# VladimirP1/rs-sync

Hardware: NVIDIA B200
Metric: presync_loss_evals_per_s (higher is better)
Workload: dtype f64

## Files before the change

rs-sync_b200/csrc/capi.cpp:

```cpp
#include "rssync_b200.h"

#include <algorithm>
#include <atomic>
#include <chrono>
#include <cmath>
#include <condition_variable>
#include <cstdio>
#include <cstdlib>
#include <cstring>
#include <functional>
#include <map>
#include <mutex>
#include <string>
#include <thread>
#include <unordered_set>
#include <utility>
#include <vector>
#if defined(__x86_64__)
#include <immintrin.h>
#endif
#if defined(__linux__)
#include <pthread.h>
#include <sched.h>
#endif
// ... 206 lines not shown
    DevBuf<unsigned> d_var_flags;
    size_t elim_n = 0;

    std::vector<rssync_problem*> replicas;
    std::vector<void*> comms;
    bool is_replica = false, owns_stream = false;
    bool force_single = false;
    uint64_t version = 0, synced_version = 0;
    DevBuf<unsigned char> d_gather;
    PinBuf<unsigned char> h_gather;
    uint64_t nccl_calls = 0, broadcast_bytes = 0;

    DevBuf<FrameDesc> d_frames;
    DevBuf<double> d_delays, d_framecost, d_costs;
    DevBuf<unsigned> d_flags;
    DevBuf<rs::PixelFrame> d_pixframes;
    DevBuf<uint64_t> d_frame_call;
    DevBuf<int> d_win_begin;
    PinBuf<double> h_pix;
    DevBuf<double> d_pix, d_stage;
    PinBuf<double> h_stage;
    std::vector<SyncLane> lanes;
    cudaEvent_t ev_sync_ready = nullptr;
    DevBuf<double> d_probe;

    std::unordered_map<int64_t, std::pair<double, double>> retime;
    DevBuf<double> d_rowq;
    DevBuf<double> d_rt_rays, d_rt_ext;
    DevBuf<int32_t> d_rt_orig, d_rt_pos;

// ... 145 lines not shown
    return RSSYNC_OK;
}

int check_grid_size(rssync_problem* p, long long F, long long D) {
    if (F * D > (1LL << 34)) { p->err = "pre-sync: grid too large"; return RSSYNC_E_INVALID; }
    return RSSYNC_OK;
}

int stage_grid(rssync_problem* p, const FrameDesc* frames, size_t n_frames, int F, const double* delays, int D,
               int curves) {
    CUDA_TRY(p, p->d_frames.reserve(std::max<size_t>(n_frames, 1)));
    CUDA_TRY(p, p->d_delays.reserve((size_t)D));
    CUDA_TRY(p, p->d_framecost.reserve((size_t)std::max(F, 1) * D));
    CUDA_TRY(p, p->d_costs.reserve((size_t)curves * D));
    CUDA_TRY(p, p->d_flags.reserve((size_t)curves * 2));
    CUDA_TRY(p, cudaMemsetAsync(p->d_flags.ptr, 0, (size_t)curves * 2 * sizeof(unsigned), p->stream));
    if (F == 0) return RSSYNC_OK;
    if (int rc = h2d(p, p->d_frames.ptr, frames, sizeof(FrameDesc) * n_frames)) return rc;
    return h2d(p, p->d_delays.ptr, delays, sizeof(double) * D);
}

int grid_max_chunk(const FrameDesc* frames, int F, const double* delays, int D, double sr, int max_n) {
    double span = 0.0;
    for (int f = 0; f < F; ++f) span = std::max(span, frames[f].ts_hi - frames[f].ts_lo);
    return rs::presync_max_chunk(delays, D, span, sr, max_n);
}

std::vector<uint64_t> call_numbers(const rssync_problem* p, const uint64_t* call_nos, int n) {
    std::vector<uint64_t> calls((size_t)n);
    for (int i = 0; i < n; ++i) calls[(size_t)i] = call_nos ? call_nos[i] : p->call_no + (uint64_t)i;
// ... 110 lines not shown
        run_end.push_back(F);
        if (run_end.size() > 16) { run_end.assign(1, F); run_dep.assign(1, (int)p->in_flight.size()); }
    } else {
        run_end.assign(1, F);
        run_dep.assign(1, 0);
    }
    const rs::DeviceData dd = p->device_data();
    if (timed) CUDA_TRY(p, cudaEventRecord(p->ev0, p->stream));
    int f0 = 0, waited = 0;
    if (run_end.size() == 1) {
        if (run_dep[0] > 0) {
            CUDA_TRY(p, cudaStreamWaitEvent(p->stream, p->in_flight[(size_t)run_dep[0] - 1].ev, 0));
            waited = run_dep[0];
        }
        rs::launch_presync_tasks(dd, p->d_frames.ptr, F, max_n, p->d_delays.ptr, n, p->seed, stream_id, call_no,
                                 idx_base, p->d_framecost.ptr, F, d_flags, p->stream, nullptr, max_chunk, p->simplified);
    } else {
        for (int k = 0; k < rssync_problem::kGridStreams; ++k) {
            if (!p->grid_stream[k]) CUDA_TRY(p, cudaStreamCreateWithFlags(&p->grid_stream[k], cudaStreamNonBlocking));
            if (!p->ev_grid[k]) CUDA_TRY(p, cudaEventCreateWithFlags(&p->ev_grid[k], cudaEventDisableTiming));
        }
        if (!p->ev_order) CUDA_TRY(p, cudaEventCreateWithFlags(&p->ev_order, cudaEventDisableTiming));
        CUDA_TRY(p, cudaEventRecord(p->ev_order, p->stream));
        for (size_t r = 0; r < run_end.size(); ++r) {
            cudaStream_t gs = p->grid_stream[r % rssync_problem::kGridStreams];
            if (r < (size_t)rssync_problem::kGridStreams) CUDA_TRY(p, cudaStreamWaitEvent(gs, p->ev_order, 0));
            if (run_dep[r] > 0) {
                CUDA_TRY(p, cudaStreamWaitEvent(gs, p->in_flight[(size_t)run_dep[r] - 1].ev, 0));
                waited = std::max(waited, run_dep[r]);
            }
            int spare = 0;
            for (size_t k = (size_t)run_dep[r]; k < p->in_flight.size(); ++k)
                if (p->in_flight[k].foreign) spare = spare_sms_for_collectives();
            rs::launch_presync_tasks(dd, p->d_frames.ptr + f0, run_end[r] - f0, max_n, p->d_delays.ptr, n, p->seed,
                                     stream_id, call_no, idx_base, p->d_framecost.ptr + f0, F, d_flags, gs,
                                     nullptr, max_chunk, p->simplified, spare);
            f0 = run_end[r];
        }
        for (int k = 0; k < rssync_problem::kGridStreams; ++k) {
            CUDA_TRY(p, cudaEventRecord(p->ev_grid[k], p->grid_stream[k]));
            CUDA_TRY(p, cudaStreamWaitEvent(p->stream, p->ev_grid[k], 0));
        }
    }
    if (timed) CUDA_TRY(p, cudaEventRecord(p->ev1, p->stream));
    if (n_launches) *n_launches = run_end.size();
    if (n_waited) *n_waited = waited;
    for (int k = 0; k < waited; ++k) p->ev_pool.push_back(p->in_flight[(size_t)k].ev);
    p->in_flight.erase(p->in_flight.begin(), p->in_flight.begin() + waited);
    return RSSYNC_OK;
}

// ... 508 lines not shown
    for (rssync_problem* r : p->replicas) r->synced_version = p->version;
    p->broadcast_bytes += p->nq * 16 * sizeof(double);
    for (const Piece& pc : pieces) p->broadcast_bytes += (pc.hi - pc.lo) * (8 * sizeof(double) + 2 * sizeof(int32_t));
    return RSSYNC_OK;
}

int grid_enqueue_rank(rssync_problem* q, const std::vector<FrameDesc>& sel, int max_n, const double* delays,
                      int cnt, uint64_t stream_id, uint64_t call_no, uint64_t idx_base, int max_chunk,
                      double* d_costs_dst, unsigned* d_flags_dst, bool timed) {
    const int F = (int)sel.size();
    CUDA_TRY(q, cudaMemsetAsync(d_flags_dst, 0, 2 * sizeof(unsigned), q->stream));
    if (cnt <= 0) return RSSYNC_OK;
    CUDA_TRY(q, q->d_frames.reserve(F));
    CUDA_TRY(q, q->d_delays.reserve(cnt));
    CUDA_TRY(q, q->d_framecost.reserve((size_t)F * cnt));
    if (int rc = h2d(q, q->d_frames.ptr, sel.data(), sizeof(FrameDesc) * F)) return rc;
    if (int rc = h2d(q, q->d_delays.ptr, delays, sizeof(double) * cnt)) return rc;
    if (int rc = enqueue_grid_kernels(q, sel, max_n, cnt, stream_id, call_no, idx_base, d_flags_dst, max_chunk, timed,
                                      nullptr, nullptr))
        return rc;
    rs::launch_presync_reduce(q->d_framecost.ptr, F, cnt, d_costs_dst, q->stream);
    CUDA_TRY(q, cudaGetLastError());
    return RSSYNC_OK;
}

int multi_presync_grid(rssync_problem* p, int64_t fb, int64_t fe, const double* delays, int n,
                       uint64_t stream_id, uint64_t call_no, uint64_t idx_base, double* costs,
                       unsigned* flags_out) {
    std::vector<FrameDesc> sel;
    int max_n = 0;
// ... 229 lines not shown
    for (int k = 0; k < rssync_problem::kGridStreams; ++k) {
        if (p->grid_stream[k]) cudaStreamDestroy(p->grid_stream[k]);
        if (p->ev_grid[k]) cudaEventDestroy(p->ev_grid[k]);
    }
    if (p->gyro_stream) { cudaStreamSynchronize(p->gyro_stream); cudaStreamDestroy(p->gyro_stream); }
    if (p->ev_gyro) cudaEventDestroy(p->ev_gyro);
    p->d_rec.release();
    p->h_gyro.release();
    p->d_gyro.release();
    p->h_rays.release(); p->d_rays.release();
    p->h_orig.release(); p->d_orig.release();
    p->h_pos.release(); p->d_pos.release();
    p->d_frames.release(); p->d_delays.release(); p->d_framecost.release(); p->d_costs.release();
    p->d_frame_call.release(); p->d_win_begin.release();
    p->h_pix.release(); p->d_pix.release(); p->d_pixframes.release(); p->d_stage.release();
    p->d_flags.release(); p->h_stage.release(); p->d_probe.release();
    p->d_gather.release(); p->h_gather.release();
    p->d_var_ts.release(); p->d_var_in.release(); p->d_var_q.release(); p->d_var_y.release(); p->d_var_rhs.release();
    p->d_var_rec.release(); p->d_var_prefix.release(); p->d_elim.release();
    p->d_var_orients.release(); p->d_var_flags.release();
    p->d_rowq.release(); p->d_rt_rays.release(); p->d_rt_ext.release(); p->d_rt_orig.release(); p->d_rt_pos.release();
    if (p->owns_stream && p->stream) { cudaStreamSynchronize(p->stream); cudaStreamDestroy(p->stream); }
    for (SyncLane& L : p->lanes) L.release();
    if (p->ev_sync_ready) cudaEventDestroy(p->ev_sync_ready);
    if (p->ev0) cudaEventDestroy(p->ev0);
    if (p->ev1) cudaEventDestroy(p->ev1);
    delete p;
}

const char* rssync_last_error(const rssync_problem* p) { return p ? p->err.c_str() : "null problem"; }

// ... 914 lines not shown
    if (!call_nos) p->call_no += (uint64_t)n;
    if (int rc = flush(p)) return rc;
    const int F = (int)all.size();
    std::vector<double> costs((size_t)n * D, 0.0);
    unsigned flags[2] = {0, 0};
    if (F > 0) {
        if (int rc = check_grid_size(p, F, D)) return rc;
        const int max_chunk = grid_max_chunk(all.data(), F, delays.data(), D, p->sr, max_n);
        if (int rc = stage_grid(p, all.data(), all.size(), F, delays.data(), D, n)) return rc;
        CUDA_TRY(p, p->d_frame_call.reserve(F));
        CUDA_TRY(p, p->d_win_begin.reserve(n + 1));
        if (int rc = h2d(p, p->d_frame_call.ptr, fcall.data(), sizeof(uint64_t) * F)) return rc;
        if (int rc = h2d(p, p->d_win_begin.ptr, wbeg.data(), sizeof(int) * (n + 1))) return rc;
        rs::launch_presync_grid(p->device_data(), p->d_frames.ptr, F, max_n, p->d_delays.ptr, D, p->seed,
                                rs::kStreamPreSync, 0, 0, p->d_framecost.ptr, p->d_costs.ptr, p->d_flags.ptr,
                                p->stream, max_chunk, p->simplified, p->d_frame_call.ptr, p->d_win_begin.ptr, n);
        if (int rc = d2h(p, costs.data(), p->d_costs.ptr, sizeof(double) * n * D)) return rc;
        if (int rc = d2h(p, flags, p->d_flags.ptr, 2 * sizeof(unsigned))) return rc;
        if (int rc = finish_stream(p, p->stream)) return rc;
        p->grid_tasks = (uint64_t)F * (uint64_t)D;
        p->grid_exact_tasks = flags[1];
    }
    if (flags[0]) { p->err = presync_panic_text(flags[0]); return RSSYNC_E_NONFINITE; }
    for (int i = 0; i < n; ++i) curve_argmin(&costs[(size_t)i * D], delays.data(), D, &out_cost[i], &out_delay[i]);
    return RSSYNC_OK;
}

int rssync_debug_presync(rssync_problem* p, double initial, int64_t fb, int64_t fe, double radius,
                         double* delays, double* costs, int point_count) {
    RS_NVTX_RANGE();
    if (!p || (point_count > 0 && (!delays || !costs))) return RSSYNC_E_INVALID;
// ... 135 lines not shown
    for (int k0 = 0; k0 < n_orient; k0 += G) {
        const int g = std::min(G, n_orient - k0);
        rs::launch_gyro_integrate(p->d_var_in.ptr, p->d_var_in.ptr + n, (int)n, &mats[(size_t)k0 * 9], g, p->d_var_orients.ptr,
                                  p->d_var_q.ptr, p->d_var_prefix.ptr, st);
        rs::launch_gyro_resample(p->d_var_ts.ptr, (int)n, p->d_var_q.ptr, g, plan.tick0, plan.rate_hz, (int)nq,
                                 p->d_var_y.ptr, p->d_var_flags.ptr + k0, st);
        rs::launch_spline_chains(p->d_var_y.ptr, p->d_elim.ptr, p->d_elim.ptr + nq, (int)nq, g, p->d_var_rhs.ptr, st);
        for (int v = 0; v < g; ++v) {
            double* rec = p->d_var_rec.ptr + (size_t)v * nq * 16;
            rs::launch_spline_finish(p->d_var_y.ptr + (size_t)v * nq * 4, p->d_var_rhs.ptr + (size_t)v * nq * 4,
                                     p->d_elim.ptr + 2 * nq, (int)nq, rec, st);
            if (F > 0) {
                dd.rec = rec;
                rs::launch_presync_grid(dd, p->d_frames.ptr, F, max_n, p->d_delays.ptr, D, p->seed, rs::kStreamPreSync,
                                        calls[(size_t)(k0 + v)], 0, p->d_framecost.ptr,
                                        p->d_costs.ptr + (size_t)(k0 + v) * D, p->d_flags.ptr + 2 * (size_t)(k0 + v), st,
                                        max_chunk, p->simplified);
            }
        }
        CUDA_TRY(p, cudaGetLastError());
        if (k0 + g >= n_orient) {
            CUDA_TRY(p, p->d_rec.reserve(nq * 16));
            CUDA_TRY(p, cudaMemcpyAsync(p->d_rec.ptr, p->d_var_rec.ptr + (size_t)(g - 1) * nq * 16, nq * 16 * sizeof(double),
                                        cudaMemcpyDeviceToDevice, st));
        }
    }
    std::vector<double> costs((size_t)n_orient * D, 0.0);
    std::vector<unsigned> resampled((size_t)n_orient, 0u), flags((size_t)n_orient * 2, 0u);
    if (F > 0)
        if (int rc = d2h(p, costs.data(), p->d_costs.ptr, costs.size() * sizeof(double))) return rc;
    if (int rc = d2h(p, resampled.data(), p->d_var_flags.ptr, resampled.size() * sizeof(unsigned))) return rc;
    if (int rc = d2h(p, flags.data(), p->d_flags.ptr, flags.size() * sizeof(unsigned))) return rc;
// ... 151 lines not shown
                retimed_bounds(rec[(size_t)f], &ext[(size_t)f * 4], readouts[j], table[f].ts_lo, table[f].ts_hi);
            }
            max_chunk[(size_t)j] = grid_max_chunk(table, F, delays.data(), D, p->sr, max_n);
        }
        if (int rc = stage_grid(p, tables.data(), tables.size(), F, delays.data(), D, n)) return rc;
        rs::DeviceData dd = p->device_data();
        dd.rays = p->d_rt_rays.ptr;
        dd.orig = p->d_rt_orig.ptr;
        dd.pos = p->d_rt_pos.ptr;
        for (int j = 0; j < n; ++j) {
            if (j > 0)
                rs::launch_retime_frames(p->d_pixframes.ptr, F, p->d_rays.ptr, p->d_orig.ptr, p->d_rowq.ptr, readouts[j],
                                         p->d_rt_rays.ptr, p->d_rt_orig.ptr, p->d_rt_pos.ptr, nullptr, st);
            rs::launch_presync_grid(dd, p->d_frames.ptr + (size_t)j * F, F, max_n, p->d_delays.ptr, D, p->seed,
                                    rs::kStreamPreSync, calls[(size_t)j], 0, p->d_framecost.ptr,
                                    p->d_costs.ptr + (size_t)j * D, p->d_flags.ptr + 2 * (size_t)j, st,
                                    max_chunk[(size_t)j], p->simplified);
        }
        if (int rc = d2h(p, costs.data(), p->d_costs.ptr, costs.size() * sizeof(double))) return rc;
        if (int rc = d2h(p, flags.data(), p->d_flags.ptr, flags.size() * sizeof(unsigned))) return rc;
        if (int rc = finish_stream(p, st)) return rc;
        p->grid_tasks = (uint64_t)F * (uint64_t)D;
        p->grid_exact_tasks = flags[(size_t)n * 2 - 1];
    }
    for (int j = 0; j < n; ++j) {
        if (const unsigned fl = flags[2 * (size_t)j]) { p->err = presync_panic_text(fl); return RSSYNC_E_NONFINITE; }
        const double* c = &costs[(size_t)j * D];
        curve_argmin(c, delays.data(), D, &out_cost[j], &out_delay[j]);
        if (out_curves) std::memcpy(out_curves + (size_t)j * D, c, sizeof(double) * D);
    }
    return RSSYNC_OK;
// ... 457 lines not shown
```

rs-sync_b200/csrc/engine.cu:

```cuda
#include "engine.h"

#include <algorithm>
#include <atomic>
#include <cmath>
#include <cstdio>
#include <map>
#include <mutex>
#include <tuple>
#include <utility>
#include <vector>

#include "device_math.cuh"
#include "gyro_scan.h"

namespace rs {

namespace {

constexpr unsigned FULL = 0xffffffffu;

#ifdef RS_CHECKED
__device__ int* g_assert_slot = nullptr;
#define RS_ASSERT(cond)                                                      \
    do {                                                                     \
// ... 860 lines not shown
#ifndef RS_GRID_RECS
#define RS_GRID_RECS 128
#endif
#ifndef RS_LOSS_UNROLL
#define RS_LOSS_UNROLL 4
#endif
#ifndef RS_GRID_GRAB
#define RS_GRID_GRAB 4
#endif
#ifndef RS_GRID_PRIOR
#define RS_GRID_PRIOR 1
#endif
#ifndef RS_PRIOR_BUMP
#define RS_PRIOR_BUMP 0x00800000u
#endif
template <int SLOTS>
struct GridCfg {
    static constexpr int kWarps = RS_GRID_WARPS;
    static constexpr int kMinBlocks = SLOTS <= 8 ? RS_GRID_MINB : 1;
    static constexpr size_t kTileBytes = (size_t)SLOTS * 2048;
    static constexpr long long kRoom = (228 * 1024) / kMinBlocks - 1024 - (long long)kLog1pTableBytes - 256 -
                                       (long long)kWarps * (long long)warp_smem_bytes(SLOTS * 32) - 2 * (long long)kTileBytes;
    static constexpr int kRecsFit = (int)(kRoom / 256 / 8 * 8);
    static constexpr int kRecs = kRecsFit < RS_GRID_RECS ? kRecsFit : RS_GRID_RECS;
    static_assert(kRecs >= 40, "grid kernel: no room for a spline window");
    static constexpr size_t kBufBytes = kTileBytes + (size_t)kRecs * 128;
    static constexpr size_t kCtlOff = kLog1pTableBytes;
    static constexpr size_t kBufOff = kCtlOff + 256;
    static constexpr size_t kWarpOff = kBufOff + 2 * kBufBytes;
    static constexpr size_t kSmem = kWarpOff + (size_t)kWarps * warp_smem_bytes(SLOTS * 32);
    static_assert(kMinBlocks * (kSmem + 1024) <= 228 * 1024, "grid kernel: shared memory over budget");
};
struct GridCtl {
    unsigned long long full[2];
    int done_a[2];
    int next_task;
    int rec_first[2], rec_cnt[2];
    int frame[2], d0[2];
    int unit[2];
    FrameDesc fd[2];
};
static_assert(sizeof(GridCtl) <= 256, "GridCtl must fit its slot");

__device__ __noinline__ void grid_stage_unit(const DeviceData& dd, const FrameDesc* frames,
                                             const double* delays, int D, int chunk, int fi, int ci, int u,
                                             GridCtl* ctl, int b, double* sTiles, double* sRec, int rec_cap) {
    const int d0 = ci * chunk;
    const int d1 = min(D, d0 + chunk);
    const FrameDesc fd = frames[fi];
    double dmin = delays[d0], dmax = dmin;
    for (int d = d0 + 1; d < d1; ++d) {
        dmin = fmin(dmin, delays[d]);
        dmax = fmax(dmax, delays[d]);
    }
    const double x_lo = ((fd.ts_lo - dd.q0) + dmin) * dd.sr, x_hi = ((fd.ts_hi - dd.q0) + dmax) * dd.sr;
    const double r_lo = floor(x_lo) - 1.0, r_hi = floor(x_hi) + 2.0;
    const bool ok = dd.sr > 0.0 && r_lo >= 0.0 && r_hi <= (double)(dd.nq - 1) && (r_hi - r_lo) < (double)rec_cap;
    const int first = ok ? (int)r_lo : 0, cnt = ok ? (int)(r_hi - r_lo) + 1 : 0;
    ctl->rec_first[b] = first;
    ctl->rec_cnt[b] = cnt;
    ctl->frame[b] = fi;
    ctl->d0[b] = d0;
    ctl->fd[b] = fd;
    __threadfence_block();
    *(volatile int*)&ctl->unit[b] = u;
    asm volatile("fence.proxy.async.shared::cta;" ::: "memory");
    const unsigned tile_bytes = (unsigned)((fd.n + 31) >> 5) * 2048u;
    const unsigned bytes = ok ? (unsigned)cnt * 128u + tile_bytes : 0u;
    mbar_arrive_expect_tx(&ctl->full[b], bytes);
    if (ok) {
        tma_load_1d(sRec, dd.rec + (size_t)first * 16, (unsigned)cnt * 128u, &ctl->full[b]);
        tma_load_1d(sTiles, dd.rays + (size_t)fd.off * 8, tile_bytes, &ctl->full[b]);
    }
}

template <int SLOTS, bool SIMPLE>
__global__ void __launch_bounds__(GridCfg<SLOTS>::kWarps * 32, GridCfg<SLOTS>::kMinBlocks)
presync_kernel(DeviceData dd, const FrameDesc* __restrict__ frames, int F,
               const double* __restrict__ delays, int D, int chunk, int cpf, uint64_t seed,
               uint64_t stream, uint64_t call_no, const uint64_t* __restrict__ frame_call_no,
               uint64_t idx_base, double* __restrict__ framecost, int cost_stride,
               unsigned* __restrict__ flags, int staged) {
    using Cfg = GridCfg<SLOTS>;
    constexpr bool simplified = SIMPLE;
    extern __shared__ __align__(128) unsigned char smem_raw[];
    constexpr int NP = SLOTS * 32;
    const int lane = threadIdx.x & 31, warp = threadIdx.x >> 5;
    double* tab = reinterpret_cast<double*>(smem_raw);
    GridCtl* ctl = reinterpret_cast<GridCtl*>(smem_raw + Cfg::kCtlOff);
    unsigned char* bufs = smem_raw + Cfg::kBufOff;
    const WarpSmem w = warp_smem(smem_raw + Cfg::kWarpOff, warp, NP);
    const long long U = (long long)F * cpf;
    const long long u_begin = U * blockIdx.x / gridDim.x;
    const int n_units = (int)(U * (blockIdx.x + 1) / gridDim.x - u_begin);
    const int fi0 = (int)(u_begin / cpf), c0 = (int)(u_begin % cpf);
    auto stage = [&](int u) {
        const int cu = c0 + u, b = u & 1;
        double* sTiles = reinterpret_cast<double*>(bufs + (size_t)b * Cfg::kBufBytes);
        grid_stage_unit(dd, frames, delays, D, chunk, fi0 + cu / cpf, cu % cpf, u, ctl, b, sTiles,
                        sTiles + SLOTS * 256, Cfg::kRecs);
    };
    if (threadIdx.x == 0) {
        mbar_init(&ctl->full[0], 1);
        mbar_init(&ctl->full[1], 1);
        ctl->done_a[0] = ctl->done_a[1] = 0;
        ctl->unit[0] = ctl->unit[1] = -1;
        ctl->next_task = 0;
        asm volatile("fence.mbarrier_init.release.cluster;" ::: "memory");
    }
    load_log1p_table(tab);
    if (threadIdx.x == 0 && staged) {
        if (n_units > 0) stage(0);
        if (n_units > 1) stage(1);
    }
    const int n_tasks = n_units * chunk;
    int cur_u = -1, rec_first = 0, rec_cnt = 0, fi = 0, d0 = 0;
    FrameDesc fd{};
    unsigned prior = 0u;
    int prior_u = -1, prior_dj = -2;
    for (int k_next = 0, k_end = 0;;) {
        if (k_next == k_end) {
            if (lane == 0) k_next = atomicAdd(&ctl->next_task, RS_GRID_GRAB);
            k_next = __shfl_sync(FULL, k_next, 0);
            k_end = min(k_next + RS_GRID_GRAB, n_tasks);
            if (k_next >= n_tasks) break;
        }
        const int k = k_next++;
        const int u = k / chunk, dj = k - u * chunk;
        const int b = u & 1;
        if (u != cur_u && !staged) {
            cur_u = u;
            const int cu = c0 + u;
            fi = fi0 + cu / cpf;
            d0 = (cu % cpf) * chunk;
            fd = frames[fi];
        } else if (u != cur_u) {
            cur_u = u;
#ifdef RS_CHECKED
            unsigned spins = 0;
#endif
            for (int have; (have = *(volatile int*)&ctl->unit[b]) != u;) {
                RS_ASSERT(++spins < (1u << 24) && have < u);
                __nanosleep(RS_POLL_NS);
            }
            const unsigned parity = (unsigned)(u >> 1) & 1u;
            while (!mbar_try_wait(&ctl->full[b], parity)) {
                RS_ASSERT(++spins < (1u << 24));
                __nanosleep(RS_POLL_NS);
            }
            RS_ASSERT(*(volatile int*)&ctl->unit[b] == u);
            rec_first = *(volatile int*)&ctl->rec_first[b];
            rec_cnt = *(volatile int*)&ctl->rec_cnt[b];
            fi = *(volatile int*)&ctl->frame[b];
            d0 = *(volatile int*)&ctl->d0[b];
            const volatile FrameDesc* vf = &ctl->fd[b];
            fd.id = vf->id; fd.off = vf->off; fd.n = vf->n; fd.ts_lo = vf->ts_lo; fd.ts_hi = vf->ts_hi;
        }
        const int di = d0 + dj;
        const bool active = di < D;
        RS_ASSERT(fi >= 0 && fi < F && dj >= 0 && dj < chunk && fd.n >= 2 && fd.n <= NP);
        double delay = 0.0;
        if (active) {
            delay = delays[di];
            const double* sTiles = reinterpret_cast<const double*>(bufs + (size_t)b * Cfg::kBufBytes);
            if (rec_cnt) build_rows_staged(dd, fd, delay, lane, w, NP, sTiles, sTiles + SLOTS * 256, rec_first, rec_cnt);
            else build_rows_global_cold(dd, fd, delay, lane, w, NP);
        }
        __syncwarp();
        if (lane == 0 && staged) {
            __threadfence_block();
            RS_ASSERT(*(volatile int*)&ctl->unit[b] == u);
            const int done = atomicAdd(&ctl->done_a[b], 1);
            RS_ASSERT(done >= 0 && done < chunk);
            if (done == chunk - 1) {
                ctl->done_a[b] = 0;
                if (u + 2 < n_units) stage(u + 2);
            }
        }
        if (!active) continue;
        const uint64_t key =
            rng_task_key(rng_prefix(seed, stream, frame_call_no ? frame_call_no[fi] : call_no,
                                    idx_base + (uint64_t)di),
                         fd.id);
        double M[3] = {0.0, 0.0, 0.0};
        unsigned bad = 0u;
        if (!simplified) {
            const bool neighbour = RS_GRID_PRIOR && prior && prior_u == u && prior_dj + 1 == dj && prior < 0x7e000000u;
            unsigned tau = 0u;
            bad = warp_ransac<SLOTS>(dd, fd, w, 20, key, lane, M, flags + 1, neighbour ? prior + RS_PRIOR_BUMP : 0u,
                                     &tau);
            prior = tau;
            prior_u = u;
            prior_dj = dj;
        }
        __syncwarp();
        constexpr int LU = RS_LOSS_UNROLL < SLOTS ? RS_LOSS_UNROLL : SLOTS;
        double ss = 0.0;
#pragma unroll 1
        for (int s0 = 0; s0 < SLOTS; s0 += LU) {
            double pm[LU];
#pragma unroll
            for (int j = 0; j < LU; ++j) {
                const int i = (s0 + j) * 32 + lane;
                pm[j] = 0.0;
                if (s0 + j < SLOTS) {
                    const double p0 = w.P[i], p1 = w.P[NP + i], p2 = w.P[2 * NP + i];
                    pm[j] = simplified ? sqrt(dot3(p0, p1, p2, p0, p1, p2)) : dot3(p0, p1, p2, M[0], M[1], M[2]);
                    w.P[i] = pm[j];
// ... 13 lines not shown
                const double r = (s0 + j < SLOTS ? w.P[(s0 + j) * 32 + lane] : 0.0) * scale;
                rho[j] = sqrt(log1p_nonneg(r * r, tab));
            }
#pragma unroll
            for (int j = 0; j < LU; ++j) acc = acc + rho[j];
        }
        const double cost = sqrt(warp_sum(acc));
        if (lane == 0) framecost[(size_t)di * cost_stride + fi] = cost;
        if (bad || !is_finite(cost)) {
            if (simplified && !is_finite(ss)) bad |= kFlagP;
            bad |= presync_diagnose(w.P, (fd.n + 31) >> 5, lane, scale, M[0], M[1], M[2], tab);
            bad = __reduce_or_sync(FULL, bad);
            if (bad && lane == 0) atomicOr(flags, bad);
        }
    }
}

__global__ void reduce_rows_kernel(const double* __restrict__ in, int rows, int cols,
                                   double* __restrict__ out) {
    const int lane = threadIdx.x & 31;
    const int row = blockIdx.x * (blockDim.x >> 5) + (threadIdx.x >> 5);
    if (row >= rows) return;
    DD acc = dd_zero();
    for (int c = lane; c < cols; c += 32) dd_add(acc, in[(size_t)row * cols + c]);
    const double v = warp_dd_sum(acc);
    if (lane == 0) out[row] = v;
}

__global__ void reduce_windows_kernel(const double* __restrict__ in, int D, int F,
                                      const int* __restrict__ win_begin, int W,
// ... 721 lines not shown
    int*& h = slots[dev];
    if (!h) {
        cudaHostAlloc((void**)&h, sizeof(int), cudaHostAllocMapped);
        *h = 0;
        int* d = nullptr;
        cudaHostGetDevicePointer((void**)&d, h, 0);
        cudaMemcpyToSymbol(g_assert_slot, &d, sizeof(d));
        return 0;
    }
    return *(volatile int*)h;
#else
    return 0;
#endif
}

uint64_t launch_count() { return g_launches.load(); }
void count_launches(uint64_t n) { g_launches += n; }

int presync_max_chunk(const double* h_delays, int D, double frame_span_s, double sample_rate, int max_n) {
    if (D <= 1) return 1;
    int recs = 0;
    RS_DISPATCH_SLOTS(max_n, { recs = GridCfg<SL>::kRecs; });
    double step = 0.0;
    for (int i = 1; i < D; ++i) step = std::max(step, std::fabs(h_delays[i] - h_delays[i - 1]));
    const double room = ((double)recs - 5.0) / sample_rate - frame_span_s;
    if (!(room > 0.0) || !(step == step)) return 1;
    if (step <= 0.0) return D;
    const double c = std::floor(room / step) + 1.0;
    return (int)std::max(1.0, std::min(c, (double)D));
}

void launch_presync_tasks(const DeviceData& dd, const FrameDesc* d_frames, int F, int max_n,
                          const double* d_delays, int D, uint64_t seed, uint64_t stream, uint64_t call_no,
                          uint64_t idx_base, double* d_framecost, int cost_stride, unsigned* d_flags,
                          cudaStream_t st, const uint64_t* d_frame_call_no, int max_chunk, bool simplified,
                          int spare_sms) {
    if (F <= 0 || D <= 0) return;
    RS_DISPATCH_SLOTS(max_n, {
        using Cfg = GridCfg<SL>;
        auto kern = simplified ? presync_kernel<SL, true> : presync_kernel<SL, false>;
        allow_smem(kern, Cfg::kSmem);
        const int sm_count = sm_count_of(current_device());
        const int per_sm = blocks_per_sm(kern, Cfg::kWarps * 32, Cfg::kSmem);
        const long long blocks_cap = (long long)std::max(1, sm_count - std::max(0, spare_sms)) * per_sm;
        int chunk = std::min(D, max_chunk > 0 ? max_chunk : Cfg::kWarps * 2);
        const long long cpf_par = (blocks_cap * 4 + F - 1) / F;
        const int chunk_par = (int)std::max<long long>(1, (D + cpf_par - 1) / cpf_par);
        chunk = std::min(chunk, std::max(chunk_par, std::min(D, Cfg::kWarps)));
        const int cpf = (D + chunk - 1) / chunk;
        chunk = (D + cpf - 1) / cpf;
        const long long units = (long long)F * cpf;
        const int grid = (int)std::max<long long>(1, std::min<long long>(units, blocks_cap));
        const int staged = chunk >= Cfg::kWarps ? 1 : 0;
        kern<<<grid, Cfg::kWarps * 32, Cfg::kSmem, st>>>(dd, d_frames, F, d_delays, D, chunk, cpf, seed, stream,
                                                         call_no, d_frame_call_no, idx_base, d_framecost,
                                                         cost_stride, d_flags, staged);
    });
    g_launches += 1;
}

void launch_presync_reduce(const double* d_framecost, int F, int D, double* d_costs, cudaStream_t st,
                           const int* d_win_begin, int n_windows) {
    if (D <= 0) return;
    if (F <= 0) {
        cudaMemsetAsync(d_costs, 0, sizeof(double) * D * (d_win_begin ? n_windows : 1), st);
        return;
    }
    if (d_win_begin)
        reduce_windows_kernel<<<(n_windows * D + 3) / 4, 128, 0, st>>>(d_framecost, D, F, d_win_begin,
                                                                      n_windows, d_costs);
    else
        reduce_rows_kernel<<<(D + 3) / 4, 128, 0, st>>>(d_framecost, D, F, d_costs);
    g_launches += 1;
}

void launch_presync_grid(const DeviceData& dd, const FrameDesc* d_frames, int F, int max_n,
                         const double* d_delays, int D, uint64_t seed, uint64_t stream,
                         uint64_t call_no, uint64_t idx_base, double* d_framecost, double* d_costs,
                         unsigned* d_flags, cudaStream_t st, int max_chunk, bool simplified,
                         const uint64_t* d_frame_call_no, const int* d_win_begin, int n_windows) {
    launch_presync_tasks(dd, d_frames, F, max_n, d_delays, D, seed, stream, call_no, idx_base, d_framecost, F,
                         d_flags, st, d_frame_call_no, max_chunk, simplified);
    launch_presync_reduce(d_framecost, F, D, d_costs, st, d_win_begin, n_windows);
}

void launch_sync_init(const DeviceData& dd, const SyncBatchDev& b, const double* d_sp_delay,
                      const uint64_t* d_sp_callno, const unsigned char* d_sp_active, uint64_t seed,
                      cudaStream_t st) {
    if (b.T <= 0) return;
    RS_DISPATCH_SLOTS(b.max_n, {
        auto kern = sync_init_kernel<SL>;
        const size_t smem = (size_t)kWarpsPerBlock * warp_smem_bytes(SL * 32);
        allow_smem(kern, smem);
        const int grid = grid_for(kern, smem, b.T);
        kern<<<grid, kWarpsPerBlock * 32, smem, st>>>(dd, b, d_sp_delay, d_sp_callno, d_sp_active, seed);
    });
    g_launches += 1;
// ... 190 lines not shown
```

rs-sync_b200/csrc/engine.h:

```cpp
#pragma once
#include <cstdint>
#include <cuda_runtime.h>

namespace rs {

constexpr int kMaxRaysPerFrame = 512;
constexpr double kNumericDiffStep = 1e-6;

struct FrameDesc {
    int64_t id;
    int32_t off;
    int32_t n;
    double ts_lo, ts_hi;
};

struct DeviceData {
    const double* rec;
    int nq;
    double q0, sr;
    const double* rays;
    const int32_t* orig;
    const int32_t* pos;
};

enum RngStream : uint64_t { kStreamPreSync = 1, kStreamDebugPreSync = 2, kStreamSyncInit = 3 };

enum : unsigned { kFlagP = 1u, kFlagM = 2u, kFlagR = 4u, kFlagRho = 8u };

void launch_presync_grid(const DeviceData& dd, const FrameDesc* d_frames, int F, int max_n,
                         const double* d_delays, int D, uint64_t seed, uint64_t stream,
                         uint64_t call_no, uint64_t idx_base, double* d_framecost, double* d_costs,
                         unsigned* d_flags, cudaStream_t st, int max_chunk, bool simplified,
                         const uint64_t* d_frame_call_no = nullptr, const int* d_win_begin = nullptr,
                         int n_windows = 0);

int presync_max_chunk(const double* h_delays, int D, double frame_span_s, double sample_rate, int max_n);

void launch_presync_tasks(const DeviceData& dd, const FrameDesc* d_frames, int F, int max_n,
                          const double* d_delays, int D, uint64_t seed, uint64_t stream, uint64_t call_no,
                          uint64_t idx_base, double* d_framecost, int cost_stride, unsigned* d_flags,
                          cudaStream_t st, const uint64_t* d_frame_call_no = nullptr, int max_chunk = 0,
                          bool simplified = false, int spare_sms = 0);
void launch_presync_reduce(const double* d_framecost, int F, int D, double* d_costs, cudaStream_t st,
                           const int* d_win_begin = nullptr, int n_windows = 0);

struct SyncTask {
    FrameDesc fd;
    int32_t sp;
    int32_t pad;
};
struct SyncBatchDev {
    const SyncTask* tasks;
    int T;
    int max_n;
    const int* sp_begin;
    int S;
    double* m;
// ... 83 lines not shown
```

Measured before the change: 33.07 billion.

## Replace static per-block unit split with global atomic work queue for presync grid

The presync kernel no longer gives each block a fixed contiguous range of (frame, chunk) units. Warps now claim units from a device-global atomic counter: whole units first, then a tail split into smaller sub-parts to balance load at the end. Staging also precomputes RNG task keys per unit in shared memory and reduces delay min/max across the warp. The cost is one global atomic per claim, an extra memset per launch, more control shared memory and more complex producer/consumer handshakes.

After: 34.41 billion, median of 6. +4.1%, better.

```diff
diff --git a/rs-sync_b200/csrc/capi.cpp b/rs-sync_b200/csrc/capi.cpp
--- a/rs-sync_b200/csrc/capi.cpp
+++ b/rs-sync_b200/csrc/capi.cpp
@@ -244,6 +244,7 @@
     DevBuf<FrameDesc> d_frames;
     DevBuf<double> d_delays, d_framecost, d_costs;
     DevBuf<unsigned> d_flags;
+    DevBuf<unsigned long long> d_queue;
     DevBuf<rs::PixelFrame> d_pixframes;
     DevBuf<uint64_t> d_frame_call;
     DevBuf<int> d_win_begin;
@@ -419,6 +420,7 @@
     CUDA_TRY(p, p->d_framecost.reserve((size_t)std::max(F, 1) * D));
     CUDA_TRY(p, p->d_costs.reserve((size_t)curves * D));
     CUDA_TRY(p, p->d_flags.reserve((size_t)curves * 2));
+    CUDA_TRY(p, p->d_queue.reserve(1 + rssync_problem::kGridStreams));
     CUDA_TRY(p, cudaMemsetAsync(p->d_flags.ptr, 0, (size_t)curves * 2 * sizeof(unsigned), p->stream));
     if (F == 0) return RSSYNC_OK;
     if (int rc = h2d(p, p->d_frames.ptr, frames, sizeof(FrameDesc) * n_frames)) return rc;
@@ -559,7 +561,8 @@
             waited = run_dep[0];
         }
         rs::launch_presync_tasks(dd, p->d_frames.ptr, F, max_n, p->d_delays.ptr, n, p->seed, stream_id, call_no,
-                                 idx_base, p->d_framecost.ptr, F, d_flags, p->stream, nullptr, max_chunk, p->simplified);
+                                 idx_base, p->d_framecost.ptr, F, d_flags, p->d_queue.ptr, p->stream, nullptr, max_chunk,
+                                 p->simplified);
     } else {
         for (int k = 0; k < rssync_problem::kGridStreams; ++k) {
             if (!p->grid_stream[k]) CUDA_TRY(p, cudaStreamCreateWithFlags(&p->grid_stream[k], cudaStreamNonBlocking));
@@ -568,7 +571,8 @@
         if (!p->ev_order) CUDA_TRY(p, cudaEventCreateWithFlags(&p->ev_order, cudaEventDisableTiming));
         CUDA_TRY(p, cudaEventRecord(p->ev_order, p->stream));
         for (size_t r = 0; r < run_end.size(); ++r) {
-            cudaStream_t gs = p->grid_stream[r % rssync_problem::kGridStreams];
+            const size_t k = r % rssync_problem::kGridStreams;
+            cudaStream_t gs = p->grid_stream[k];
             if (r < (size_t)rssync_problem::kGridStreams) CUDA_TRY(p, cudaStreamWaitEvent(gs, p->ev_order, 0));
             if (run_dep[r] > 0) {
                 CUDA_TRY(p, cudaStreamWaitEvent(gs, p->in_flight[(size_t)run_dep[r] - 1].ev, 0));
@@ -578,8 +582,8 @@
             for (size_t k = (size_t)run_dep[r]; k < p->in_flight.size(); ++k)
                 if (p->in_flight[k].foreign) spare = spare_sms_for_collectives();
             rs::launch_presync_tasks(dd, p->d_frames.ptr + f0, run_end[r] - f0, max_n, p->d_delays.ptr, n, p->seed,
-                                     stream_id, call_no, idx_base, p->d_framecost.ptr + f0, F, d_flags, gs,
-                                     nullptr, max_chunk, p->simplified, spare);
+                                     stream_id, call_no, idx_base, p->d_framecost.ptr + f0, F, d_flags,
+                                     p->d_queue.ptr + 1 + k, gs, nullptr, max_chunk, p->simplified, spare);
             f0 = run_end[r];
         }
         for (int k = 0; k < rssync_problem::kGridStreams; ++k) {
@@ -1118,6 +1122,7 @@
     CUDA_TRY(q, q->d_frames.reserve(F));
     CUDA_TRY(q, q->d_delays.reserve(cnt));
     CUDA_TRY(q, q->d_framecost.reserve((size_t)F * cnt));
+    CUDA_TRY(q, q->d_queue.reserve(1 + rssync_problem::kGridStreams));
     if (int rc = h2d(q, q->d_frames.ptr, sel.data(), sizeof(FrameDesc) * F)) return rc;
     if (int rc = h2d(q, q->d_delays.ptr, delays, sizeof(double) * cnt)) return rc;
     if (int rc = enqueue_grid_kernels(q, sel, max_n, cnt, stream_id, call_no, idx_base, d_flags_dst, max_chunk, timed,
@@ -1377,7 +1382,7 @@
     p->d_frames.release(); p->d_delays.release(); p->d_framecost.release(); p->d_costs.release();
     p->d_frame_call.release(); p->d_win_begin.release();
     p->h_pix.release(); p->d_pix.release(); p->d_pixframes.release(); p->d_stage.release();
-    p->d_flags.release(); p->h_stage.release(); p->d_probe.release();
+    p->d_flags.release(); p->d_queue.release(); p->h_stage.release(); p->d_probe.release();
     p->d_gather.release(); p->h_gather.release();
     p->d_var_ts.release(); p->d_var_in.release(); p->d_var_q.release(); p->d_var_y.release(); p->d_var_rhs.release();
     p->d_var_rec.release(); p->d_var_prefix.release(); p->d_elim.release();
@@ -2322,7 +2327,8 @@
         if (int rc = h2d(p, p->d_win_begin.ptr, wbeg.data(), sizeof(int) * (n + 1))) return rc;
         rs::launch_presync_grid(p->device_data(), p->d_frames.ptr, F, max_n, p->d_delays.ptr, D, p->seed,
                                 rs::kStreamPreSync, 0, 0, p->d_framecost.ptr, p->d_costs.ptr, p->d_flags.ptr,
-                                p->stream, max_chunk, p->simplified, p->d_frame_call.ptr, p->d_win_begin.ptr, n);
+                                p->d_queue.ptr, p->stream, max_chunk, p->simplified, p->d_frame_call.ptr,
+                                p->d_win_begin.ptr, n);
         if (int rc = d2h(p, costs.data(), p->d_costs.ptr, sizeof(double) * n * D)) return rc;
         if (int rc = d2h(p, flags, p->d_flags.ptr, 2 * sizeof(unsigned))) return rc;
         if (int rc = finish_stream(p, p->stream)) return rc;
@@ -2488,8 +2494,8 @@
                 dd.rec = rec;
                 rs::launch_presync_grid(dd, p->d_frames.ptr, F, max_n, p->d_delays.ptr, D, p->seed, rs::kStreamPreSync,
                                         calls[(size_t)(k0 + v)], 0, p->d_framecost.ptr,
-                                        p->d_costs.ptr + (size_t)(k0 + v) * D, p->d_flags.ptr + 2 * (size_t)(k0 + v), st,
-                                        max_chunk, p->simplified);
+                                        p->d_costs.ptr + (size_t)(k0 + v) * D, p->d_flags.ptr + 2 * (size_t)(k0 + v),
+                                        p->d_queue.ptr, st, max_chunk, p->simplified);
             }
         }
         CUDA_TRY(p, cudaGetLastError());
@@ -2671,7 +2677,7 @@
                                          p->d_rt_rays.ptr, p->d_rt_orig.ptr, p->d_rt_pos.ptr, nullptr, st);
             rs::launch_presync_grid(dd, p->d_frames.ptr + (size_t)j * F, F, max_n, p->d_delays.ptr, D, p->seed,
                                     rs::kStreamPreSync, calls[(size_t)j], 0, p->d_framecost.ptr,
-                                    p->d_costs.ptr + (size_t)j * D, p->d_flags.ptr + 2 * (size_t)j, st,
+                                    p->d_costs.ptr + (size_t)j * D, p->d_flags.ptr + 2 * (size_t)j, p->d_queue.ptr, st,
                                     max_chunk[(size_t)j], p->simplified);
         }
         if (int rc = d2h(p, costs.data(), p->d_costs.ptr, costs.size() * sizeof(double))) return rc;
diff --git a/rs-sync_b200/csrc/engine.cu b/rs-sync_b200/csrc/engine.cu
--- a/rs-sync_b200/csrc/engine.cu
+++ b/rs-sync_b200/csrc/engine.cu
@@ -898,45 +898,95 @@
 #ifndef RS_PRIOR_BUMP
 #define RS_PRIOR_BUMP 0x00800000u
 #endif
+constexpr int kUnitCap = 64;
+constexpr size_t kCtlBytes = 256 + 2 * kUnitCap * sizeof(uint64_t);
 template <int SLOTS>
 struct GridCfg {
     static constexpr int kWarps = RS_GRID_WARPS;
     static constexpr int kMinBlocks = SLOTS <= 8 ? RS_GRID_MINB : 1;
     static constexpr size_t kTileBytes = (size_t)SLOTS * 2048;
-    static constexpr long long kRoom = (228 * 1024) / kMinBlocks - 1024 - (long long)kLog1pTableBytes - 256 -
+    static constexpr long long kRoom = (228 * 1024) / kMinBlocks - 1024 - (long long)kLog1pTableBytes - (long long)kCtlBytes -
                                        (long long)kWarps * (long long)warp_smem_bytes(SLOTS * 32) - 2 * (long long)kTileBytes;
     static constexpr int kRecsFit = (int)(kRoom / 256 / 8 * 8);
     static constexpr int kRecs = kRecsFit < RS_GRID_RECS ? kRecsFit : RS_GRID_RECS;
     static_assert(kRecs >= 40, "grid kernel: no room for a spline window");
     static constexpr size_t kBufBytes = kTileBytes + (size_t)kRecs * 128;
     static constexpr size_t kCtlOff = kLog1pTableBytes;
-    static constexpr size_t kBufOff = kCtlOff + 256;
+    static constexpr size_t kBufOff = kCtlOff + kCtlBytes;
     static constexpr size_t kWarpOff = kBufOff + 2 * kBufBytes;
     static constexpr size_t kSmem = kWarpOff + (size_t)kWarps * warp_smem_bytes(SLOTS * 32);
     static_assert(kMinBlocks * (kSmem + 1024) <= 228 * 1024, "grid kernel: shared memory over budget");
 };
+static_assert(GridCfg<7>::kRecs == 128, "grid kernel: the C2 shape keeps its 128-record window");
 struct GridCtl {
     unsigned long long full[2];
-    int done_a[2];
-    int next_task;
+    unsigned long long word[2];
+    int left_a[2];
     int rec_first[2], rec_cnt[2];
     int frame[2], d0[2];
-    int unit[2];
+    int tail;
     FrameDesc fd[2];
 };
 static_assert(sizeof(GridCtl) <= 256, "GridCtl must fit its slot");
 
-__device__ __noinline__ void grid_stage_unit(const DeviceData& dd, const FrameDesc* frames,
-                                             const double* delays, int D, int chunk, int fi, int ci, int u,
-                                             GridCtl* ctl, int b, double* sTiles, double* sRec, int rec_cap) {
-    const int d0 = ci * chunk;
-    const int d1 = min(D, d0 + chunk);
+struct GridQueue {
+    unsigned long long* next;
+    long long head, claims;
+    int chunk, cpf, parts, sub;
+};
+
+__device__ __forceinline__ void grid_claim_range(const GridQueue& q, int D, long long c, int& fi, int& d0, int& len) {
+    const bool whole = c < q.head;
+    const long long u = whole ? c : q.head + (c - q.head) / q.parts;
+    const int part = whole ? 0 : (int)((c - q.head) % q.parts);
+    fi = (int)(u / q.cpf);
+    const int ud0 = (int)(u % q.cpf) * q.chunk, ud1 = min(D, ud0 + q.chunk);
+    d0 = ud0 + part * (whole ? q.chunk : q.sub);
+    len = max(0, min(ud1, d0 + (whole ? q.chunk : q.sub)) - d0);
+}
+
+struct GridKeys {
+    uint64_t seed, stream, call_no, idx_base;
+    const uint64_t* frame_call_no;
+};
+
+__device__ __noinline__ void grid_stage_unit(const DeviceData& dd, const FrameDesc* frames, const double* delays,
+                                             int D, const GridQueue& q, const GridKeys& gk, unsigned seq,
+                                             GridCtl* ctl, uint64_t* sKeys, double* sTiles, double* sRec,
+                                             int rec_cap) {
+    const int lane = threadIdx.x & 31, b = (int)(seq & 1u);
+    long long c = 0;
+    int fi = 0, d0 = 0, len = 0;
+    for (;;) {
+        if (lane == 0) c = (long long)atomicAdd(q.next, 1ull);
+        c = __shfl_sync(FULL, c, 0);
+        if (c >= q.claims) break;
+        grid_claim_range(q, D, c, fi, d0, len);
+        if (len > 0) break;
+    }
+    if (len == 0) {
+        if (lane == 0) {
+            ctl->tail = 1;
+            atomicExch(&ctl->word[b], (unsigned long long)seq << 32);
+        }
+        return;
+    }
+    RS_ASSERT(fi >= 0 && d0 >= 0 && len <= kUnitCap && d0 + len <= D);
     const FrameDesc fd = frames[fi];
-    double dmin = delays[d0], dmax = dmin;
-    for (int d = d0 + 1; d < d1; ++d) {
-        dmin = fmin(dmin, delays[d]);
-        dmax = fmax(dmax, delays[d]);
-    }
+    const uint64_t call_no = gk.frame_call_no ? gk.frame_call_no[fi] : gk.call_no;
+    double dmin = INFINITY, dmax = -INFINITY;
+    for (int d = lane; d < len; d += 32) {
+        sKeys[d] = rng_task_key(rng_prefix(gk.seed, gk.stream, call_no, gk.idx_base + (uint64_t)(d0 + d)), fd.id);
+        const double x = delays[d0 + d];
+        dmin = fmin(dmin, x);
+        dmax = fmax(dmax, x);
+    }
+    for (int o = 16; o > 0; o >>= 1) {
+        dmin = fmin(dmin, __shfl_xor_sync(FULL, dmin, o));
+        dmax = fmax(dmax, __shfl_xor_sync(FULL, dmax, o));
+    }
+    __syncwarp();
+    if (lane != 0) return;
     const double x_lo = ((fd.ts_lo - dd.q0) + dmin) * dd.sr, x_hi = ((fd.ts_hi - dd.q0) + dmax) * dd.sr;
     const double r_lo = floor(x_lo) - 1.0, r_hi = floor(x_hi) + 2.0;
     const bool ok = dd.sr > 0.0 && r_lo >= 0.0 && r_hi <= (double)(dd.nq - 1) && (r_hi - r_lo) < (double)rec_cap;
@@ -946,8 +996,7 @@
     ctl->frame[b] = fi;
     ctl->d0[b] = d0;
     ctl->fd[b] = fd;
-    __threadfence_block();
-    *(volatile int*)&ctl->unit[b] = u;
+    ctl->left_a[b] = len;
     asm volatile("fence.proxy.async.shared::cta;" ::: "memory");
     const unsigned tile_bytes = (unsigned)((fd.n + 31) >> 5) * 2048u;
     const unsigned bytes = ok ? (unsigned)cnt * 128u + tile_bytes : 0u;
@@ -956,15 +1005,26 @@
         tma_load_1d(sRec, dd.rec + (size_t)first * 16, (unsigned)cnt * 128u, &ctl->full[b]);
         tma_load_1d(sTiles, dd.rays + (size_t)fd.off * 8, tile_bytes, &ctl->full[b]);
     }
-}
+    __threadfence_block();
+    atomicExch(&ctl->word[b], ((unsigned long long)seq << 32) | ((unsigned long long)len << 24));
+}
+
+#ifdef RS_GRID_TRACE
+constexpr int kGridTraceWords = 2 + 2 * RS_GRID_WARPS;
+__device__ unsigned long long* g_grid_trace = nullptr;
+__device__ unsigned g_grid_trace_blocks = 0;
+__device__ __forceinline__ unsigned long long global_timer() {
+    unsigned long long t;
+    asm volatile("mov.u64 %0, %%globaltimer;" : "=l"(t));
+    return t;
+}
+#endif
 
 template <int SLOTS, bool SIMPLE>
 __global__ void __launch_bounds__(GridCfg<SLOTS>::kWarps * 32, GridCfg<SLOTS>::kMinBlocks)
 presync_kernel(DeviceData dd, const FrameDesc* __restrict__ frames, int F,
-               const double* __restrict__ delays, int D, int chunk, int cpf, uint64_t seed,
-               uint64_t stream, uint64_t call_no, const uint64_t* __restrict__ frame_call_no,
-               uint64_t idx_base, double* __restrict__ framecost, int cost_stride,
-               unsigned* __restrict__ flags, int staged) {
+               const double* __restrict__ delays, int D, GridQueue q, GridKeys gk,
+               double* __restrict__ framecost, int cost_stride, unsigned* __restrict__ flags, int staged) {
     using Cfg = GridCfg<SLOTS>;
     constexpr bool simplified = SIMPLE;
     extern __shared__ __align__(128) unsigned char smem_raw[];
@@ -972,110 +1032,151 @@
     const int lane = threadIdx.x & 31, warp = threadIdx.x >> 5;
     double* tab = reinterpret_cast<double*>(smem_raw);
     GridCtl* ctl = reinterpret_cast<GridCtl*>(smem_raw + Cfg::kCtlOff);
+    uint64_t* keys = reinterpret_cast<uint64_t*>(smem_raw + Cfg::kCtlOff + 256);
     unsigned char* bufs = smem_raw + Cfg::kBufOff;
     const WarpSmem w = warp_smem(smem_raw + Cfg::kWarpOff, warp, NP);
-    const long long U = (long long)F * cpf;
-    const long long u_begin = U * blockIdx.x / gridDim.x;
-    const int n_units = (int)(U * (blockIdx.x + 1) / gridDim.x - u_begin);
-    const int fi0 = (int)(u_begin / cpf), c0 = (int)(u_begin % cpf);
-    auto stage = [&](int u) {
-        const int cu = c0 + u, b = u & 1;
+#ifdef RS_GRID_TRACE
+    unsigned long long* trace =
+        blockIdx.x < g_grid_trace_blocks ? g_grid_trace + (size_t)blockIdx.x * kGridTraceWords : nullptr;
+    unsigned trace_tasks = 0;
+    if (trace && threadIdx.x == 0) {
+        unsigned sm;
+        asm volatile("mov.u32 %0, %%smid;" : "=r"(sm));
+        trace[0] = sm;
+        trace[1] = global_timer();
+    }
+#endif
+    auto stage = [&](unsigned seq) {
+        const int b = (int)(seq & 1u);
         double* sTiles = reinterpret_cast<double*>(bufs + (size_t)b * Cfg::kBufBytes);
-        grid_stage_unit(dd, frames, delays, D, chunk, fi0 + cu / cpf, cu % cpf, u, ctl, b, sTiles,
-                        sTiles + SLOTS * 256, Cfg::kRecs);
+        grid_stage_unit(dd, frames, delays, D, q, gk, seq, ctl, keys + b * kUnitCap, sTiles, sTiles + SLOTS * 256,
+                        Cfg::kRecs);
     };
     if (threadIdx.x == 0) {
         mbar_init(&ctl->full[0], 1);
         mbar_init(&ctl->full[1], 1);
-        ctl->done_a[0] = ctl->done_a[1] = 0;
-        ctl->unit[0] = ctl->unit[1] = -1;
-        ctl->next_task = 0;
+        ctl->tail = 0;
         asm volatile("fence.mbarrier_init.release.cluster;" ::: "memory");
     }
+    __syncwarp();
+    if (warp == 0 && staged) {
+        stage(0u);
+        stage(1u);
+    }
     load_log1p_table(tab);
-    if (threadIdx.x == 0 && staged) {
-        if (n_units > 0) stage(0);
-        if (n_units > 1) stage(1);
-    }
-    const int n_tasks = n_units * chunk;
-    int cur_u = -1, rec_first = 0, rec_cnt = 0, fi = 0, d0 = 0;
+    unsigned u = 0u;
+    unsigned grab = 0u;
+    int fi = 0, d0 = 0;
     FrameDesc fd{};
     unsigned prior = 0u;
-    int prior_u = -1, prior_dj = -2;
-    for (int k_next = 0, k_end = 0;;) {
-        if (k_next == k_end) {
-            if (lane == 0) k_next = atomicAdd(&ctl->next_task, RS_GRID_GRAB);
-            k_next = __shfl_sync(FULL, k_next, 0);
-            k_end = min(k_next + RS_GRID_GRAB, n_tasks);
-            if (k_next >= n_tasks) break;
-        }
-        const int k = k_next++;
-        const int u = k / chunk, dj = k - u * chunk;
-        const int b = u & 1;
-        if (u != cur_u && !staged) {
-            cur_u = u;
-            const int cu = c0 + u;
-            fi = fi0 + cu / cpf;
-            d0 = (cu % cpf) * chunk;
-            fd = frames[fi];
-        } else if (u != cur_u) {
-            cur_u = u;
+    for (;;) {
+        if ((grab & 0xffu) == (grab >> 8)) {
+            if (staged) {
+                unsigned long long got = 0ull;
+                if (lane == 0) {
 #ifdef RS_CHECKED
-            unsigned spins = 0;
+                    unsigned spins = 0;
 #endif
-            for (int have; (have = *(volatile int*)&ctl->unit[b]) != u;) {
-                RS_ASSERT(++spins < (1u << 24) && have < u);
-                __nanosleep(RS_POLL_NS);
+                    for (;;) {
+                        const int p = (int)(u & 1u);
+                        const unsigned long long cur = *(volatile unsigned long long*)&ctl->word[p];
+                        const unsigned seq = (unsigned)(cur >> 32);
+                        const int clen = (int)((cur >> 24) & 0xffu), taken = (int)(cur & 0xffffffu);
+                        if (clen == 0 && (int)(u - seq) >= 0) {
+                            const unsigned long long other = *(volatile unsigned long long*)&ctl->word[p ^ 1];
+                            if (((other >> 24) & 0xffu) == 0u) break;
+                            ++u;
+                            continue;
+                        }
+                        if ((int)(seq - u) < 0) {
+                            RS_ASSERT(++spins < (1u << 24));
+                            __nanosleep(RS_POLL_NS);
+                            continue;
+                        }
+                        if (seq != u || taken >= clen) {
+                            ++u;
+                            continue;
+                        }
+                        const int g = *(volatile int*)&ctl->tail ? 1 : RS_GRID_GRAB;
+                        if (atomicCAS(&ctl->word[p], cur, cur + (unsigned long long)g) == cur) {
+                            got = ((unsigned long long)u << 32) | ((unsigned long long)clen << 24) |
+                                  ((unsigned long long)min(clen, taken + g) << 8) | (unsigned long long)taken;
+                            break;
+                        }
+                    }
+                }
+                got = __shfl_sync(FULL, got, 0);
+                if (got == 0ull) break;
+                u = (unsigned)(got >> 32);
+                grab = (unsigned)got & 0xffffu;
+                const int b = (int)(u & 1u);
+#ifdef RS_CHECKED
+                unsigned spins = 0;
+#endif
+                while (!mbar_try_wait(&ctl->full[b], (u >> 1) & 1u)) {
+                    RS_ASSERT(++spins < (1u << 24));
+                    __nanosleep(RS_POLL_NS);
+                }
+                fi = *(volatile int*)&ctl->frame[b];
+                d0 = *(volatile int*)&ctl->d0[b];
+                const volatile FrameDesc* vf = &ctl->fd[b];
+                fd.id = vf->id; fd.off = vf->off; fd.n = vf->n; fd.ts_lo = vf->ts_lo; fd.ts_hi = vf->ts_hi;
+            } else {
+                long long c = 0;
+                if (lane == 0) c = (long long)atomicAdd(q.next, 1ull);
+                c = __shfl_sync(FULL, c, 0);
+                if (c >= q.claims) break;
+                int len;
+                grid_claim_range(q, D, c, fi, d0, len);
+                u = (unsigned)c;
+                grab = (unsigned)len << 8;
+                if (len == 0) continue;
+                fd = frames[fi];
             }
-            const unsigned parity = (unsigned)(u >> 1) & 1u;
-            while (!mbar_try_wait(&ctl->full[b], parity)) {
-                RS_ASSERT(++spins < (1u << 24));
-                __nanosleep(RS_POLL_NS);
+            prior = 0u;
+        }
+        const int b = (int)(u & 1u);
+        const int dt = (int)(grab++ & 0xffu);
+#ifdef RS_GRID_TRACE
+        ++trace_tasks;
+#endif
+        const int di = d0 + dt;
+        RS_ASSERT(fi >= 0 && fi < F && dt >= 0 && dt < (int)(grab >> 8) && di < D && fd.n >= 2 && fd.n <= NP);
+        RS_ASSERT(!staged || (unsigned)(*(volatile unsigned long long*)&ctl->word[b] >> 32) == u);
+        const double delay = delays[di];
+        if (staged) {
+            const double* sTiles = reinterpret_cast<const double*>(bufs + (size_t)b * Cfg::kBufBytes);
+            const int rec_cnt = *(volatile int*)&ctl->rec_cnt[b];
+            if (rec_cnt)
+                build_rows_staged(dd, fd, delay, lane, w, NP, sTiles, sTiles + SLOTS * 256,
+                                  *(volatile int*)&ctl->rec_first[b], rec_cnt);
+            else build_rows_global_cold(dd, fd, delay, lane, w, NP);
+        } else {
+            build_rows_global_cold(dd, fd, delay, lane, w, NP);
+        }
+        const uint64_t key = staged ? *(volatile uint64_t*)&keys[b * kUnitCap + dt]
+                                    : rng_task_key(rng_prefix(gk.seed, gk.stream,
+                                                              gk.frame_call_no ? gk.frame_call_no[fi] : gk.call_no,
+                                                              gk.idx_base + (uint64_t)di),
+                                                   fd.id);
+        __syncwarp();
+        if (staged) {
+            int left = 0;
+            if (lane == 0) {
+                __threadfence_block();
+                left = atomicSub(&ctl->left_a[b], 1);
+                RS_ASSERT(left >= 1 && left <= kUnitCap);
             }
-            RS_ASSERT(*(volatile int*)&ctl->unit[b] == u);
-            rec_first = *(volatile int*)&ctl->rec_first[b];
-            rec_cnt = *(volatile int*)&ctl->rec_cnt[b];
-            fi = *(volatile int*)&ctl->frame[b];
-            d0 = *(volatile int*)&ctl->d0[b];
-            const volatile FrameDesc* vf = &ctl->fd[b];
-            fd.id = vf->id; fd.off = vf->off; fd.n = vf->n; fd.ts_lo = vf->ts_lo; fd.ts_hi = vf->ts_hi;
-        }
-        const int di = d0 + dj;
-        const bool active = di < D;
-        RS_ASSERT(fi >= 0 && fi < F && dj >= 0 && dj < chunk && fd.n >= 2 && fd.n <= NP);
-        double delay = 0.0;
-        if (active) {
-            delay = delays[di];
-            const double* sTiles = reinterpret_cast<const double*>(bufs + (size_t)b * Cfg::kBufBytes);
-            if (rec_cnt) build_rows_staged(dd, fd, delay, lane, w, NP, sTiles, sTiles + SLOTS * 256, rec_first, rec_cnt);
-            else build_rows_global_cold(dd, fd, delay, lane, w, NP);
-        }
-        __syncwarp();
-        if (lane == 0 && staged) {
-            __threadfence_block();
-            RS_ASSERT(*(volatile int*)&ctl->unit[b] == u);
-            const int done = atomicAdd(&ctl->done_a[b], 1);
-            RS_ASSERT(done >= 0 && done < chunk);
-            if (done == chunk - 1) {
-                ctl->done_a[b] = 0;
-                if (u + 2 < n_units) stage(u + 2);
-            }
-        }
-        if (!active) continue;
-        const uint64_t key =
-            rng_task_key(rng_prefix(seed, stream, frame_call_no ? frame_call_no[fi] : call_no,
-                                    idx_base + (uint64_t)di),
-                         fd.id);
+            if (__shfl_sync(FULL, left, 0) == 1) stage(u + 2u);
+        }
         double M[3] = {0.0, 0.0, 0.0};
         unsigned bad = 0u;
         if (!simplified) {
-            const bool neighbour = RS_GRID_PRIOR && prior && prior_u == u && prior_dj + 1 == dj && prior < 0x7e000000u;
+            const bool neighbour = RS_GRID_PRIOR && prior && prior < 0x7e000000u;
             unsigned tau = 0u;
             bad = warp_ransac<SLOTS>(dd, fd, w, 20, key, lane, M, flags + 1, neighbour ? prior + RS_PRIOR_BUMP : 0u,
                                      &tau);
             prior = tau;
-            prior_u = u;
-            prior_dj = dj;
         }
         __syncwarp();
         constexpr int LU = RS_LOSS_UNROLL < SLOTS ? RS_LOSS_UNROLL : SLOTS;
@@ -1119,6 +1220,12 @@
             if (bad && lane == 0) atomicOr(flags, bad);
         }
     }
+#ifdef RS_GRID_TRACE
+    if (trace && lane == 0) {
+        trace[2 + warp] = global_timer();
+        trace[2 + Cfg::kWarps + warp] = trace_tasks;
+    }
+#endif
 }
 
 __global__ void reduce_rows_kernel(const double* __restrict__ in, int rows, int cols,
@@ -1870,6 +1977,15 @@
 #endif
 }
 
+#ifdef RS_GRID_TRACE
+extern "C" int rssync_debug_grid_trace(unsigned long long* d_buf, unsigned blocks) {
+    if (!d_buf) blocks = 0;
+    if (cudaMemcpyToSymbol(g_grid_trace, &d_buf, sizeof(d_buf)) != cudaSuccess) return -1;
+    if (cudaMemcpyToSymbol(g_grid_trace_blocks, &blocks, sizeof(blocks)) != cudaSuccess) return -1;
+    return kGridTraceWords;
+}
+#endif
+
 uint64_t launch_count() { return g_launches.load(); }
 void count_launches(uint64_t n) { g_launches += n; }
 
@@ -1889,8 +2005,8 @@
 void launch_presync_tasks(const DeviceData& dd, const FrameDesc* d_frames, int F, int max_n,
                           const double* d_delays, int D, uint64_t seed, uint64_t stream, uint64_t call_no,
                           uint64_t idx_base, double* d_framecost, int cost_stride, unsigned* d_flags,
-                          cudaStream_t st, const uint64_t* d_frame_call_no, int max_chunk, bool simplified,
-                          int spare_sms) {
+                          unsigned long long* d_queue, cudaStream_t st, const uint64_t* d_frame_call_no,
+                          int max_chunk, bool simplified, int spare_sms) {
     if (F <= 0 || D <= 0) return;
     RS_DISPATCH_SLOTS(max_n, {
         using Cfg = GridCfg<SL>;
@@ -1899,17 +2015,23 @@
         const int sm_count = sm_count_of(current_device());
         const int per_sm = blocks_per_sm(kern, Cfg::kWarps * 32, Cfg::kSmem);
         const long long blocks_cap = (long long)std::max(1, sm_count - std::max(0, spare_sms)) * per_sm;
-        int chunk = std::min(D, max_chunk > 0 ? max_chunk : Cfg::kWarps * 2);
+        int chunk = std::min(std::min(D, kUnitCap), max_chunk > 0 ? max_chunk : Cfg::kWarps * 2);
         const long long cpf_par = (blocks_cap * 4 + F - 1) / F;
         const int chunk_par = (int)std::max<long long>(1, (D + cpf_par - 1) / cpf_par);
-        chunk = std::min(chunk, std::max(chunk_par, std::min(D, Cfg::kWarps)));
+        chunk = std::min(chunk, std::max(chunk_par, std::min(std::min(D, kUnitCap), Cfg::kWarps)));
         const int cpf = (D + chunk - 1) / chunk;
         chunk = (D + cpf - 1) / cpf;
         const long long units = (long long)F * cpf;
         const int grid = (int)std::max<long long>(1, std::min<long long>(units, blocks_cap));
         const int staged = chunk >= Cfg::kWarps ? 1 : 0;
-        kern<<<grid, Cfg::kWarps * 32, Cfg::kSmem, st>>>(dd, d_frames, F, d_delays, D, chunk, cpf, seed, stream,
-                                                         call_no, d_frame_call_no, idx_base, d_framecost,
+        GridQueue q{d_queue, units, units, chunk, cpf, 1, chunk};
+        q.parts = staged ? std::max(1, chunk / Cfg::kWarps) : (chunk + RS_GRID_GRAB - 1) / RS_GRID_GRAB;
+        q.sub = (chunk + q.parts - 1) / q.parts;
+        q.head = staged ? units - std::min<long long>(units, grid) : 0;
+        q.claims = q.head + (units - q.head) * q.parts;
+        const GridKeys gk{seed, stream, call_no, idx_base, d_frame_call_no};
+        cudaMemsetAsync(d_queue, 0, sizeof(unsigned long long), st);
+        kern<<<grid, Cfg::kWarps * 32, Cfg::kSmem, st>>>(dd, d_frames, F, d_delays, D, q, gk, d_framecost,
                                                          cost_stride, d_flags, staged);
     });
     g_launches += 1;
@@ -1933,10 +2055,10 @@
 void launch_presync_grid(const DeviceData& dd, const FrameDesc* d_frames, int F, int max_n,
                          const double* d_delays, int D, uint64_t seed, uint64_t stream,
                          uint64_t call_no, uint64_t idx_base, double* d_framecost, double* d_costs,
-                         unsigned* d_flags, cudaStream_t st, int max_chunk, bool simplified,
-                         const uint64_t* d_frame_call_no, const int* d_win_begin, int n_windows) {
+                         unsigned* d_flags, unsigned long long* d_queue, cudaStream_t st, int max_chunk,
+                         bool simplified, const uint64_t* d_frame_call_no, const int* d_win_begin, int n_windows) {
     launch_presync_tasks(dd, d_frames, F, max_n, d_delays, D, seed, stream, call_no, idx_base, d_framecost, F,
-                         d_flags, st, d_frame_call_no, max_chunk, simplified);
+                         d_flags, d_queue, st, d_frame_call_no, max_chunk, simplified);
     launch_presync_reduce(d_framecost, F, D, d_costs, st, d_win_begin, n_windows);
 }
 
diff --git a/rs-sync_b200/csrc/engine.h b/rs-sync_b200/csrc/engine.h
--- a/rs-sync_b200/csrc/engine.h
+++ b/rs-sync_b200/csrc/engine.h
@@ -30,7 +30,8 @@
 void launch_presync_grid(const DeviceData& dd, const FrameDesc* d_frames, int F, int max_n,
                          const double* d_delays, int D, uint64_t seed, uint64_t stream,
                          uint64_t call_no, uint64_t idx_base, double* d_framecost, double* d_costs,
-                         unsigned* d_flags, cudaStream_t st, int max_chunk, bool simplified,
+                         unsigned* d_flags, unsigned long long* d_queue, cudaStream_t st, int max_chunk,
+                         bool simplified,
                          const uint64_t* d_frame_call_no = nullptr, const int* d_win_begin = nullptr,
                          int n_windows = 0);
 
@@ -39,8 +40,8 @@
 void launch_presync_tasks(const DeviceData& dd, const FrameDesc* d_frames, int F, int max_n,
                           const double* d_delays, int D, uint64_t seed, uint64_t stream, uint64_t call_no,
                           uint64_t idx_base, double* d_framecost, int cost_stride, unsigned* d_flags,
-                          cudaStream_t st, const uint64_t* d_frame_call_no = nullptr, int max_chunk = 0,
-                          bool simplified = false, int spare_sms = 0);
+                          unsigned long long* d_queue, cudaStream_t st, const uint64_t* d_frame_call_no = nullptr,
+                          int max_chunk = 0, bool simplified = false, int spare_sms = 0);
 void launch_presync_reduce(const double* d_framecost, int F, int D, double* d_costs, cudaStream_t st,
                            const int* d_win_begin = nullptr, int n_windows = 0);
 
```
